# Jittor/JDet

Hardware: AMD Instinct MI355X
Metric: img/s S2ANet-R50-FPN train step, 1024x1024 synthetic tiles (higher is better)
Workload: dtype f32; 1 GPU; s2anet_train; model=S2ANet-R50-FPN (configs/s2anet/s2anet_r50_fpn_1x_dota.py), global_batch=2, tile=1024x1024, gts_per_image=64, optimizer=SGD mom 0.9 wd 1e-4 clip 35 + StepLR warm-up (the config's lr), parallelism=dp1 (DDP, RCCL all-reduce)

## Files before the change

### jdet_amd/_lib.py

```python
import ctypes
import os
import subprocess

import torch

_HERE = os.path.dirname(os.path.abspath(__file__))
CSRC = os.path.join(_HERE, "csrc")
LIB_PATH = os.path.join(CSRC, "libjdet_hip.so")

_i, _f, _p, _sz, _l = ctypes.c_int, ctypes.c_float, ctypes.c_void_p, ctypes.c_size_t, ctypes.c_long



class BnParams(ctypes.Structure):
    _fields_ = [("weight", _p), ("bias", _p), ("mean", _p), ("var", _p), ("eps", _f)]


class ConvEpilogue(ctypes.Structure):
    _fields_ = [("mode", _i), ("affine", _i), ("relu", _i), ("bn", BnParams), ("residual", _p), ("grad_out", _p),
                ("act", _p), ("sums", _p)]


class BnSumsJob(ctypes.Structure):
    _fields_ = [("partial", _p), ("rows", _l), ("C", _i), ("gamma", _p), ("grad_gamma", _p), ("grad_beta", _p)]
# ... 85 lines not shown
                                      _p, _p, _p, _sz, _p]),
    "jdet_level_pack_nhwc": (_i, [_p, _p, _p, _i, _i, _i, _i, _i, _p, _p]),
    "jdet_align_conv_offset": (_i, [_p, _i, _i, _i, _f, _i, _p, _p]),
    "jdet_frozen_bn_act_forward": (_i, [_p, _p, _l, _i, _p, _p, _p, _p, _f, _i, _p, _p]),
    "jdet_frozen_bn_act_backward_workspace": (_sz, [_l, _i]),
    "jdet_frozen_bn_act_backward": (_i, [_p, _p, _p, _l, _i, _p, _p, _p, _p, _f, _i, _p, _p, _p, _p, _p, _sz, _p]),
    "jdet_bias_act_backward": (_i, [_p, _p, _l, _i, _i, _p, _p, _p, _sz, _p]),
    "jdet_channel_sum_workspace": (_sz, [_l, _i]),
    "jdet_channel_sum": (_i, [_p, _l, _i, _p, _p, _sz, _p]),
    "jdet_arf_forward": (_i, [_p, _p] + [_i] * 6 + [_p, _p]),
    "jdet_arf_backward": (_i, [_p, _p] + [_i] * 6 + [_p, _p]),
    "jdet_arf_forward_cl": (_i, [_p, _p] + [_i] * 6 + [_p, _p]),
    "jdet_arf_backward_cl": (_i, [_p, _p] + [_i] * 6 + [_p, _p]),
    "jdet_rip_forward": (_i, [_p, _l, _i, _i, _p, _p]),
    "jdet_rip_backward": (_i, [_p, _p, _p, _l, _i, _i, _p, _p]),
    "jdet_delta2bbox_rotated": (_i, [_p, _p, _i, _i, _p, _p, _f, _p, _p]),
    "jdet_bbox2delta_rotated": (_i, [_p, _p, _i, _p, _p, _p, _p]),
    "jdet_midpoint_offset_decode": (_i, [_p, _p, _l, _p, _p, _f, _p, _p]),
    "jdet_midpoint_offset_encode": (_i, [_p, _p, _l, _p, _p, _p, _p]),
    "jdet_oriented_delta_decode": (_i, [_p, _p, _l, _i, _p, _p, _f, _p, _p]),
    "jdet_oriented_delta_encode": (_i, [_p, _p, _l, _p, _p, _p, _p]),
    "jdet_gliding_targets": (_i, [_p, _p, _l, _p, _p, _p, _p, _p, _p]),
    "jdet_gliding_decode": (_i, [_p, _p, _p, _p, _l, _i, _p, _p, _f, _f, _f, _f, _p, _p, _p]),
    "jdet_gv_delta_encode": (_i, [_p, _p, _l, _p, _p, _p, _p]),
    "jdet_gv_delta_decode": (_i, [_p, _p, _l, _i, _p, _p, _f, _f, _f, _p, _p]),
    "jdet_anchor_targets_rotated": (_i, [_p, _p, _p, _p, _i, _i, _p, _p, _f, _p, _p, _p, _p, _p, _p]),
    "jdet_anchor_targets_rotated_boxes": (_i, [_p, _p, _p, _i, _i, _f, _p, _p, _p, _p, _p, _p]),
    "jdet_obb2hbb2obb": (_i, [_p, _i, _i, _p, _p]),
    "jdet_assign_max_iou_workspace": (_sz, [_i]),
    "jdet_assign_max_iou": (_i, [_p, _i, _i, _f, _f, _f, _f, _i, _i, _p, _i, _p, _p, _p, _p, _sz, _p]),
}

ATSS_SIGNATURES = {
    "jdet_atss_assign_workspace": (_sz, [_i, _i, _i, _i]),
    "jdet_atss_assign": (_i, [_p, _i, _i, _p, _i, _p, _i, _p, _p, _i, _i, _p, _p, _p, _p, _sz, _p]),
}

ROWS_SIGNATURES = {
    "jdet_rows_nonzero_workspace": (_sz, [_i, _i, _i]),
    "jdet_rows_nonzero": (_i, [_p, _i, _i, _i, _i, _p, _p, _p, _p, _p, _sz, _p]),
    "jdet_conv3x3_rows_supported": (_i, [_i, _i]),
    "jdet_conv3x3_wgrad_rows_workers": (_i, [_i, _i]),
    "jdet_conv3x3_wgrad_rows": (_i, [_p, _p, _p, _p, _i, _i, _i, _i, _i, _p, _p]),
    "jdet_conv3x3_dgrad_rows": (_i, [_p, _p, _p, _p, _i, _i, _i, _i, _i, _i, _p, _p]),
}

ROWS_FWD_SIGNATURES = {
    "jdet_rows_from_flags_workspace": (_sz, [_i, _i, _i]),
    "jdet_rows_from_flags": (_i, [_p, _i, _i, _i, _p, _p, _p, _p, _p, _sz, _p]),
    "jdet_conv3x3_rows_forward_supported": (_i, [_i, _i]),
    "jdet_conv3x3_rows_forward": (_i, [_p, _p, _p, _i, _p, _p, _p, _i, _i, _i, _i, _i, _i, _p, _p]),
}

FCOS_SIGNATURES = {
    "jdet_fcos_targets": (_i, [_p, _p, _i, _p, _p, _p, _i, _i, _i, _i, _i, _f, _p, _p, _p, _p, _p]),
    "jdet_poly_iou_loss": (_i, [_p, _p, _p, _l, _i, _f, _p, _p, _p]),
}

REPPOINTS_SIGNATURES = {
    "jdet_convex_point_assign_workspace": (_sz, [_i, _i]),
    "jdet_convex_point_assign": (_i, [_p, _i, _i, _p, _p, _i, _p, _p, _p, _i, _i, _f, _i, _i, _p, _p, _p, _sz, _p]),
    "jdet_convex_giou_loss": (_i, [_p, _p, _p, _p, _l, _p, _p, _p]),
}

H2RBOX_SIGNATURES = {
    "jdet_rotate_crop": (_i, [_p, _i, _i, _i, _i, _i, _i, _f, _f, _i, _p, _p]),
    "jdet_h2rbox_aug_loss_forward": (_i, [_p, _i, _p, _p, _p, _p, _p, _i, _i, _f, _f, _f, _i, _i, _f, _f, _f, _p, _p, _p]),
    "jdet_h2rbox_aug_loss_backward": (_i, [_p, _i, _p, _p, _p, _p, _p, _i, _i, _f, _f, _f, _i, _i, _f, _f, _f, _p, _p, _p,
                                           _p, _p, _p, _p, _p]),
}

_lib = None

REFERENCE_SORT = 0


def build(force=False, verbose=False):
    cmd = ["make", "-C", CSRC, "-j8"] + (["-B"] if force else [])
    r = subprocess.run(cmd, capture_output=True, text=True)
    if r.returncode != 0:
        raise RuntimeError("building libjdet_hip.so failed:\n" + r.stdout[-4000:] + r.stderr[-4000:])
    if verbose:
        print(r.stdout[-2000:])
    return LIB_PATH


def lib():
    global _lib
    if _lib is None:
        if not os.path.exists(LIB_PATH):
            raise RuntimeError(
                "jdet_amd: %s not found.  Build it with `python -c 'import __graft_entry__ as g; g.build()'` "
                "or `make -C jdet_amd/csrc` (needs hipcc).  There is no CPU fallback." % LIB_PATH)
        l = ctypes.CDLL(LIB_PATH)
        for name, (res, args) in list(SIGNATURES.items()) + list(ATSS_SIGNATURES.items()) + list(ROWS_SIGNATURES.items()) + \
                list(ROWS_FWD_SIGNATURES.items()) + list(FCOS_SIGNATURES.items()) + list(REPPOINTS_SIGNATURES.items()) + \
                list(H2RBOX_SIGNATURES.items()):
            fn = getattr(l, name)
            fn.restype = res
            fn.argtypes = args
        _lib = l
    return _lib


class JDetHipError(RuntimeError):
    pass


_ERR = {-1: "bad argument", -2: "unsupported shape", -3: "workspace too small"}


def check(status, what):
    if status != 0:
        msg = _ERR.get(status, "hipError_t %d" % status)
        raise JDetHipError("%s failed: %s" % (what, msg))


def stream_ptr(t=None):
    if t is not None and t.is_cuda and t.device.index != torch.cuda.current_device():
        torch.cuda.set_device(t.device)
    return torch.cuda.current_stream(t.device if t is not None else None).cuda_stream


def need_device(*tensors):
    for t in tensors:
        if t is None:
            continue
        if not t.is_cuda:
            raise JDetHipError(
                "jdet_amd ops run only on a HIP device (got a %s tensor); there is no CPU fallback "
                "in the product path" % t.device)


def f32c(t):
    if t.dtype != torch.float32:
        t = t.float()
    return t.contiguous()


def vec5(v):
    return (ctypes.c_float * 5)(*[float(x) for x in v])


def vecn(v, n):
    v = [float(x) for x in v]
    assert len(v) == n
    return (ctypes.c_float * n)(*v)


def ptr(t):
# ... 33 lines not shown
```

### jdet_amd/csrc/conv_rows.hip

```cpp
#include "conv_mfma.h"
#include "jdet_hip_rows.h"
#include "jdet_hip_rows_fwd.h"

namespace {

constexpr int kBlk = 256;
constexpr int kFlagRows = 64;

typedef unsigned v4u __attribute__((ext_vector_type(4)));

__global__ __launch_bounds__(256) void rows_flag_kernel(const float* __restrict__ g, long P, int C4,
                                                        uint8_t* __restrict__ flags) {
  const int lane = threadIdx.x & 63, wave = threadIdx.x >> 6;
  const long base = (long)blockIdx.x * kFlagRows + wave * (kFlagRows / 4);
  const v4u* g4 = reinterpret_cast<const v4u*>(g);
  for (int r = 0; r < kFlagRows / 4; r += 4) {
    unsigned acc[4] = {0u, 0u, 0u, 0u};
#pragma unroll
    for (int u = 0; u < 4; u++) {
      const long row = base + r + u;
      if (row < P)
        for (int c = lane; c < C4; c += 64) {
          const v4u v = g4[row * C4 + c];
          acc[u] |= (v[0] | v[1] | v[2] | v[3]) & 0x7fffffffu;
        }
    }
#pragma unroll
    for (int u = 0; u < 4; u++) {
      const long row = base + r + u;
      const bool any = __ballot(acc[u] != 0u) != 0ull;
      if (lane == 0 && row < P) flags[row] = any ? 1 : 0;
    }
  }
}

__device__ __forceinline__ int wave_sum(int v) {
#pragma unroll
  for (int o = 32; o > 0; o >>= 1) v += __shfl_xor(v, o, 64);
  return v;
}

__global__ __launch_bounds__(256) void rows_dilate_kernel(const uint8_t* __restrict__ flags, int H, int W, long P,
                                                          uint8_t* __restrict__ dflags, int* __restrict__ cnt,
                                                          int* __restrict__ dcnt) {
  __shared__ int s_sum[2][4];
  const int tid = threadIdx.x, lane = tid & 63, wave = tid >> 6;
  const long p = (long)blockIdx.x * kBlk + tid;
  bool f = false, d = false;
  if (p < P) {
    f = flags[p] != 0;
    const unsigned hw = (unsigned)(H * W), up = (unsigned)p;
    const unsigned rem = up - (up / hw) * hw;
    const int y = (int)(rem / (unsigned)W), x = (int)(rem - (unsigned)y * (unsigned)W);
#pragma unroll
    for (int dy = -1; dy <= 1; dy++)
// ... 189 lines not shown
#pragma unroll
    for (int q = 0; q < BK / 2; q++) {
      if (q + 1 < BK / 2) frags(q + 1);
#pragma unroll
      for (int i = 0; i < TM; i++)
#pragma unroll
        for (int j = 0; j < TN; j++)
          acc[i][j] = __builtin_amdgcn_mfma_f32_32x32x2f32(fa[q & 1][i], fb[q & 1][j], acc[i][j], 0, 0, 0);
    }
    store_step(buf ^ 1);
    __syncthreads();
  }

  const long gw_bytes = (long)a.Cout * 9 * a.Cin * 4;
  if (m0 + BM <= a.Cout && n0 + BN <= a.Cin && gw_bytes < (1L << 32)) {
    const __amdgpu_buffer_rsrc_t rgw = __builtin_amdgcn_make_buffer_rsrc((void*)a.gw, 0, (unsigned)gw_bytes, 0x00020000);
    const unsigned row_bytes = (unsigned)(9 * a.Cin * 4);
#pragma unroll
    for (int i = 0; i < TM; i++)
#pragma unroll
      for (int j = 0; j < TN; j++) {
        const unsigned ci = (unsigned)(n0 + wn * 32 * TN + j * 32 + (lane & 31));
        const unsigned co = (unsigned)(m0 + wm * 32 * TM + i * 32 + 4 * (lane >> 5));
        const unsigned base = ((co * 9u + (unsigned)tap) * (unsigned)a.Cin + ci) * 4u;
#pragma unroll
        for (int e = 0; e < 16; e++)
          __builtin_amdgcn_raw_ptr_buffer_atomic_fadd_f32(acc[i][j][e], rgw, (int)base, (int)(cd_row(e) * row_bytes), 0);
      }
    return;
  }
#pragma unroll
  for (int i = 0; i < TM; i++)
#pragma unroll
    for (int j = 0; j < TN; j++) {
      const int ci = n0 + wn * 32 * TN + j * 32 + (lane & 31);
#pragma unroll
      for (int e = 0; e < 16; e++) {
        const int co = m0 + wm * 32 * TM + i * 32 + cd_row(e) + 4 * (lane >> 5);
        if (co < a.Cout && ci < a.Cin) unsafeAtomicAdd(a.gw + ((size_t)co * 9 + tap) * a.Cin + ci, acc[i][j][e]);
      }
    }
}

struct DgradRowsArgs {
  const float* g;
  const float* wd;
  const int* rows;
  const int* count;
  float* gx;
  int N, H, W, Cin, Cout;
  const float* bias;
  const float* rowmask;
  int relu;
};

template <int BK, int KG, bool FWD>
__global__ __launch_bounds__(256 * KG) __attribute__((amdgpu_waves_per_eu(4)))
void conv3x3_dgrad_rows_kernel(DgradRowsArgs a) {
  constexpr int BT = 64;
  constexpr int DEPTH = KG >= 1 ? 1 : 2;
  using TL = MfmaTile<BT, BK, KG>;
  constexpr int T = TL::T, CH = TL::CH, RPP = TL::RPP, PASSES = TL::PASSES, TILE = TL::TILE, QN = TL::QN;
  static_assert(T == 1, "64 x 64 tile");
  __shared__ __attribute__((aligned(16))) char s_raw[4 * TILE];
  const int tid = threadIdx.x, lane = tid & 63, wave = tid >> 6;
  const int P = a.N * a.H * a.W;
  const int KC = a.Cout, NO = a.Cin;
  int cnt = a.count[0];
  cnt = cnt < 0 ? 0 : (cnt > P ? P : cnt);
  const int NT = (NO + BT - 1) / BT;
  const int mtile = (int)((unsigned)blockIdx.x / (unsigned)NT);
  const int m0 = mtile * BT;
  if (m0 >= cnt) return;
  const int n0 = (blockIdx.x - mtile * NT) * BT;
  const __amdgpu_buffer_rsrc_t rx =
      __builtin_amdgcn_make_buffer_rsrc((void*)a.g, 0, (unsigned)((long)P * KC * 4), 0x00020000);
  const __amdgpu_buffer_rsrc_t rw =
      __builtin_amdgcn_make_buffer_rsrc((void*)a.wd, 0, (unsigned)((long)NO * 9 * KC * 4), 0x00020000);
  const int lchunk = tid % CH, lrow = tid / CH;
  int img[PASSES], py[PASSES], px[PASSES];
  bool m_ok[PASSES];
  unsigned wv[PASSES];
  int st_off[PASSES];
  const unsigned hw = (unsigned)(a.H * a.W);
#pragma unroll
  for (int p = 0; p < PASSES; p++) {
    const int row = p * RPP + lrow;
    const int li = m0 + row;
    const unsigned pos = li < cnt ? (unsigned)a.rows[li] : 0xFFFFFFFFu;
    m_ok[p] = pos < (unsigned)P;
    const unsigned im = m_ok[p] ? pos / hw : 0u, rem = m_ok[p] ? pos - im * hw : 0u, oy = rem / (unsigned)a.W;
    img[p] = (int)im;
    py[p] = (int)oy;
    px[p] = (int)(rem - oy * (unsigned)a.W);
    wv[p] = n0 + row < NO ? ((unsigned)((n0 + row) * 9 * KC + lchunk * 4)) * 4u : kOob;
    st_off[p] = swz_bytes<BK>(row, lchunk);
  }
  const int nsteps = 9 * (KC / BK);

  unsigned av[PASSES];
  auto set_tap = [&](int tap) {
    const int r = (tap * 11) >> 5, s = tap - r * 3;
#pragma unroll
    for (int p = 0; p < PASSES; p++) {
      const int yy = py[p] + r - 1, xx = px[p] + s - 1;
      const bool in = m_ok[p] && (unsigned)yy < (unsigned)a.H && (unsigned)xx < (unsigned)a.W;
      const unsigned off = ((unsigned)(((img[p] * a.H + yy) * a.W + xx) * KC + lchunk * 4)) * 4u;
      av[p] = in ? off : kOob;
    }
  };

  v4f ra[DEPTH][PASSES], rb[DEPTH][PASSES];
  auto load_set = [&](auto setc, int tap, int c) {
    constexpr int S = decltype(setc)::value;
    const unsigned sa = (unsigned)(c * 4), sb = (unsigned)((tap * KC + c) * 4);
#pragma unroll
    for (int p = 0; p < PASSES; p++) {
      ra[S][p] = buf_load(rx, av[p], sa);
      rb[S][p] = buf_load(rw, wv[p], sb);
    }
  };
  auto store_set = [&](auto setc, int buf) {
    constexpr int S = decltype(setc)::value;
#pragma unroll
    for (int p = 0; p < PASSES; p++) {
      *reinterpret_cast<v4f*>(s_raw + buf * 2 * TILE + st_off[p]) = ra[S][p];
      *reinterpret_cast<v4f*>(s_raw + buf * 2 * TILE + TILE + st_off[p]) = rb[S][p];
    }
  };
  auto load_step = [&](int tap, int c) { load_set(Set0{}, tap, c); };
  auto store_step = [&](int buf) { store_set(Set0{}, buf); };

  const int kg = wave >> 2, wm = (wave >> 1) & 1, wn = wave & 1;
  const int frow = lane & 31, fhalf = lane >> 5;
  int fa_off[QN], fb_off[QN];
#pragma unroll
  for (int qq = 0; qq < QN; qq++) {
    const int chunk = (qq * KG + kg) * 2 + fhalf;
    fa_off[qq] = swz_bytes<BK>(wm * (BT / 2) + frow, chunk);
    fb_off[qq] = TILE + swz_bytes<BK>(wn * (BT / 2) + frow, chunk);
  }
  v16f acc[T][T];
#pragma unroll
  for (int e = 0; e < 16; e++) acc[0][0][e] = 0.f;

  int tap = 0, c = 0;
  set_tap(0);
  auto advance = [&]() {
    c += BK;
    if (c == KC) {
      c = 0;
      tap++;
      set_tap(tap);
    }
  };
  auto mfma_step = [&](int buf) { ::mfma_step<BT, BK, KG>(s_raw, buf, fa_off, fb_off, acc); };
#include "conv_mfma_loop.inc"
  if (KG == 2) {
    float* red = reinterpret_cast<float*>(s_raw);
    if (kg == 1) {
#pragma unroll
      for (int e = 0; e < 16; e++) red[red_index<T>(wave, lane, 0, 0, e)] = acc[0][0][e];
    }
    __syncthreads();
    if (kg == 1) return;
  }

  const __amdgpu_buffer_rsrc_t ry =
      __builtin_amdgcn_make_buffer_rsrc((void*)a.gx, 0, (unsigned)((long)P * NO * 4), 0x00020000);
  const int lrow0 = m0 + wm * (BT / 2) + 4 * (lane >> 5);
  const int n = n0 + wn * (BT / 2) + (lane & 31);
  unsigned dst[16];
  float mk[16];
  float b = 0.f;
  if constexpr (FWD) b = (a.bias && n < NO) ? a.bias[n] : 0.f;
#pragma unroll
  for (int e = 0; e < 16; e++) {
    const int li = lrow0 + cd_row(e);
    const unsigned pos = li < cnt ? (unsigned)a.rows[li] : 0xFFFFFFFFu;
    dst[e] = (pos < (unsigned)P && n < NO) ? (pos * (unsigned)NO + (unsigned)n) * 4u : kOob;
    if constexpr (FWD) mk[e] = (a.rowmask && pos < (unsigned)P) ? a.rowmask[pos] : 1.f;
  }
#pragma unroll
  for (int e = 0; e < 16; e++) {
    float v = acc[0][0][e];
    if (KG == 2) v += reinterpret_cast<const float*>(s_raw)[red_index<T>(wave, lane, 0, 0, e)];
    if constexpr (FWD) {
      v += b;
      if (a.relu) v = fmaxf(v, 0.f);
      if (a.rowmask) v *= mk[e];
    }
    __builtin_amdgcn_raw_buffer_store_b32(__builtin_bit_cast(unsigned, v), ry, dst[e], 0u, 0);
  }
}

inline size_t align16(size_t v) { return (v + 15) & ~(size_t)15; }

inline int wgrad_rows_workers(int Cin, int Cout) {
  const int tm = Cout > 64 ? 2 : 1;
  const long tiles = (long)((Cout + 64 * tm - 1) / (64 * tm)) * ((Cin + 63) / 64) * 9;
  long kw = 1152 / tiles;
  return (int)(kw < 8 ? 8 : (kw > 64 ? 64 : kw));
}

}

JDET_API size_t jdet_rows_nonzero_workspace(int N, int H, int W) {
  if (N <= 0 || H <= 0 || W <= 0) return 0;
  const long P = (long)N * H * W;
  const long nb = (P + kBlk - 1) / kBlk;
  return align16((size_t)P) + sizeof(int32_t) * 2 * (size_t)nb;
}

JDET_API int jdet_rows_nonzero(const float* g_nhwc, int N, int H, int W, int C, uint8_t* flags, int32_t* rows,
                               int32_t* rows_dilated, int32_t* counts, void* workspace, size_t workspace_bytes,
                               jdet_stream_t stream) {
  if (N <= 0 || H <= 0 || W <= 0 || C <= 0) return JDET_E_BADARG;
  if (C % 4 != 0) return JDET_E_UNSUPPORTED;
  const long P = (long)N * H * W;
  if (P * C >= (1L << 30)) return JDET_E_UNSUPPORTED;
  if (!g_nhwc || !flags || !rows || !rows_dilated || !counts) return JDET_E_BADARG;
  if (((uintptr_t)g_nhwc & 15) || (((uintptr_t)rows | (uintptr_t)rows_dilated | (uintptr_t)counts) & 3))
    return JDET_E_BADARG;
  if (!workspace || workspace_bytes < jdet_rows_nonzero_workspace(N, H, W)) return JDET_E_WORKSPACE;
  if ((uintptr_t)workspace & 3) return JDET_E_BADARG;
  hipStream_t st = (hipStream_t)stream;
  const unsigned nb = (unsigned)((P + kBlk - 1) / kBlk);
  uint8_t* dflags = (uint8_t*)workspace;
  int* cnt = (int*)((char*)workspace + align16((size_t)P));
  int* dcnt = cnt + nb;
  hipLaunchKernelGGL(rows_flag_kernel, dim3((unsigned)((P + kFlagRows - 1) / kFlagRows)), dim3(256), 0, st, g_nhwc, P,
                     C / 4, flags);
  hipLaunchKernelGGL(rows_dilate_kernel, dim3(nb), dim3(256), 0, st, flags, H, W, P, dflags, cnt, dcnt);
  hipLaunchKernelGGL(rows_list_kernel, dim3(nb), dim3(256), 0, st, flags, dflags, P, cnt, dcnt, rows, rows_dilated,
                     counts);
  return jdet_launch_status();
}

JDET_API int jdet_conv3x3_rows_supported(int Cin, int Cout) {
  return Cin > 0 && Cout > 0 && Cin % 4 == 0 && Cout % 16 == 0;
}

JDET_API int jdet_conv3x3_wgrad_rows_workers(int Cin, int Cout) {
  return jdet_conv3x3_rows_supported(Cin, Cout) ? wgrad_rows_workers(Cin, Cout) : 0;
}

JDET_API int jdet_conv3x3_wgrad_rows(const float* x_nhwc, const float* gy_nhwc, const int32_t* rows,
                                     const int32_t* count, int N, int H, int W, int Cin, int Cout, float* gw_krsc,
                                     jdet_stream_t stream) {
  if (N <= 0 || H <= 0 || W <= 0 || Cin <= 0 || Cout <= 0) return JDET_E_BADARG;
  if (!jdet_conv3x3_rows_supported(Cin, Cout)) return JDET_E_UNSUPPORTED;
  const long P = (long)N * H * W;
  if ((P + BKW) * (Cin > Cout ? Cin : Cout) >= (1L << 30)) return JDET_E_UNSUPPORTED;
  if (!x_nhwc || !gy_nhwc || !rows || !count || !gw_krsc) return JDET_E_BADARG;
  if ((((uintptr_t)x_nhwc) | ((uintptr_t)gy_nhwc)) & 15 || (((uintptr_t)rows | (uintptr_t)count) & 3)) return JDET_E_BADARG;
  const int tm = Cout > 64 ? 2 : 1;
  const int kw = wgrad_rows_workers(Cin, Cout);
  const unsigned grid = (unsigned)(((Cout + 64 * tm - 1) / (64 * tm)) * ((Cin + 63) / 64) * 9 * kw);
  WgradRowsArgs a{x_nhwc, gy_nhwc, rows, count, gw_krsc, N, H, W, Cin, Cout, kw};
  hipStream_t st = (hipStream_t)stream;
  if (tm == 2) hipLaunchKernelGGL((conv3x3_wgrad_rows_kernel<2>), dim3(grid), dim3(256), 0, st, a);
  else hipLaunchKernelGGL((conv3x3_wgrad_rows_kernel<1>), dim3(grid), dim3(256), 0, st, a);
  return jdet_launch_status();
}

JDET_API int jdet_conv3x3_dgrad_rows(const float* gy_nhwc, const float* wd_crsk, const int32_t* rows,
                                     const int32_t* count, int N, int H, int W, int Cin, int Cout, int zero_first,
                                     float* gx_nhwc, jdet_stream_t stream) {
  if (N <= 0 || H <= 0 || W <= 0 || Cin <= 0 || Cout <= 0) return JDET_E_BADARG;
  if (!jdet_conv3x3_rows_supported(Cin, Cout)) return JDET_E_UNSUPPORTED;
  const long P = (long)N * H * W;
  if (P * (Cin > Cout ? Cin : Cout) >= (1L << 30)) return JDET_E_UNSUPPORTED;
  if (!gy_nhwc || !wd_crsk || !rows || !count || !gx_nhwc) return JDET_E_BADARG;
  if ((((uintptr_t)gy_nhwc) | ((uintptr_t)wd_crsk)) & 15 || (((uintptr_t)rows | (uintptr_t)count | (uintptr_t)gx_nhwc) & 3))
    return JDET_E_BADARG;
  hipStream_t st = (hipStream_t)stream;
  if (zero_first) {
    const int e = jdet_zero_async(gx_nhwc, sizeof(float) * (size_t)P * Cin, st);
    if (e) return e;
  }
  DgradRowsArgs a{gy_nhwc, wd_crsk, rows, count, gx_nhwc, N, H, W, Cin, Cout, nullptr, nullptr, 0};
  const unsigned grid = (unsigned)(((P + 63) / 64) * ((Cin + 63) / 64));
  if (Cout % 32 == 0) hipLaunchKernelGGL((conv3x3_dgrad_rows_kernel<32, 2, false>), dim3(grid), dim3(512), 0, st, a);
  else hipLaunchKernelGGL((conv3x3_dgrad_rows_kernel<16, 1, false>), dim3(grid), dim3(256), 0, st, a);
  return jdet_launch_status();
}


JDET_API size_t jdet_rows_from_flags_workspace(int N, int H, int W) {
  if (N <= 0 || H <= 0 || W <= 0) return 0;
  const long P = (long)N * H * W;
  const long nb = (P + kBlk - 1) / kBlk;
  return 2 * align16((size_t)P) + sizeof(int32_t) * 4 * (size_t)nb;
}

JDET_API int jdet_rows_from_flags(const uint8_t* flags, int N, int H, int W, int32_t* rows, int32_t* rows_dilated,
                                  int32_t* rows_dilated2, int32_t* counts, void* workspace, size_t workspace_bytes,
                                  jdet_stream_t stream) {
  if (N <= 0 || H <= 0 || W <= 0) return JDET_E_BADARG;
  const long P = (long)N * H * W;
  if (P >= (1L << 30)) return JDET_E_UNSUPPORTED;
  if (!flags || !rows || !rows_dilated || !rows_dilated2 || !counts) return JDET_E_BADARG;
  if (((uintptr_t)rows | (uintptr_t)rows_dilated | (uintptr_t)rows_dilated2 | (uintptr_t)counts) & 3) return JDET_E_BADARG;
  if (!workspace || workspace_bytes < jdet_rows_from_flags_workspace(N, H, W)) return JDET_E_WORKSPACE;
  if ((uintptr_t)workspace & 3) return JDET_E_BADARG;
  hipStream_t st = (hipStream_t)stream;
  const unsigned nb = (unsigned)((P + kBlk - 1) / kBlk);
  uint8_t* d1 = (uint8_t*)workspace;
  uint8_t* d2 = d1 + align16((size_t)P);
  int* c0 = (int*)(d2 + align16((size_t)P));
  int* c1 = c0 + nb;
  int* c1b = c1 + nb;
  int* c2 = c1b + nb;
  hipLaunchKernelGGL(rows_dilate_kernel, dim3(nb), dim3(256), 0, st, flags, H, W, P, d1, c0, c1);
  hipLaunchKernelGGL(rows_dilate_kernel, dim3(nb), dim3(256), 0, st, (const uint8_t*)d1, H, W, P, d2, c1b, c2);
  hipLaunchKernelGGL(rows_list_kernel, dim3(nb), dim3(256), 0, st, flags, (const uint8_t*)d1, P, (const int*)c0,
                     (const int*)c1, rows, rows_dilated, counts);
  hipLaunchKernelGGL(rows_list_kernel, dim3(nb), dim3(256), 0, st, (const uint8_t*)d1, (const uint8_t*)d2, P,
                     (const int*)c1b, (const int*)c2, rows_dilated, rows_dilated2, counts + 1);
  return jdet_launch_status();
}

JDET_API int jdet_conv3x3_rows_forward_supported(int Cin, int Cout) {
  return Cin > 0 && Cout > 0 && Cin % 16 == 0 && Cout % 16 == 0;
}

JDET_API int jdet_conv3x3_rows_forward(const float* x_nhwc, const float* w_krsc, const float* bias, int relu,
                                       const float* rowmask, const int32_t* rows, const int32_t* count, int N, int H,
                                       int W, int Cin, int Cout, int zero_first, float* y_nhwc, jdet_stream_t stream) {
  if (N <= 0 || H <= 0 || W <= 0 || Cin <= 0 || Cout <= 0) return JDET_E_BADARG;
  if (!jdet_conv3x3_rows_forward_supported(Cin, Cout)) return JDET_E_UNSUPPORTED;
  const long P = (long)N * H * W;
  if (P * (Cin > Cout ? Cin : Cout) >= (1L << 30)) return JDET_E_UNSUPPORTED;
  if (!x_nhwc || !w_krsc || !rows || !count || !y_nhwc) return JDET_E_BADARG;
  if ((((uintptr_t)x_nhwc) | ((uintptr_t)w_krsc)) & 15) return JDET_E_BADARG;
  if (((uintptr_t)rows | (uintptr_t)count | (uintptr_t)y_nhwc | (uintptr_t)bias | (uintptr_t)rowmask) & 3) return JDET_E_BADARG;
  hipStream_t st = (hipStream_t)stream;
  if (zero_first) {
    const int e = jdet_zero_async(y_nhwc, sizeof(float) * (size_t)P * Cout, st);
    if (e) return e;
  }
  DgradRowsArgs a{x_nhwc, w_krsc, rows, count, y_nhwc, N, H, W, Cout, Cin, bias, rowmask, relu ? 1 : 0};
  const unsigned grid = (unsigned)(((P + 63) / 64) * ((Cout + 63) / 64));
  if (Cin % 32 == 0) hipLaunchKernelGGL((conv3x3_dgrad_rows_kernel<32, 2, true>), dim3(grid), dim3(512), 0, st, a);
  else hipLaunchKernelGGL((conv3x3_dgrad_rows_kernel<16, 1, true>), dim3(grid), dim3(256), 0, st, a);
  return jdet_launch_status();
}
```

### jdet_amd/ops/conv_igemm.py

```python
import os
import weakref

import torch

from jdet_amd import _lib as L


def supported(cin, cout):
    return bool(L.lib().jdet_conv3x3_igemm_supported(int(cin), int(cout)))


def weight_krsc(weight):
    return L.f32c(weight.permute(0, 2, 3, 1))


def conv3x3_nhwc(x_nhwc, w_krsc, bias=None, relu=False, rowmask=None, offset=None, tile=0):
    L.need_device(x_nhwc, w_krsc, bias, rowmask, offset)
    N, H, W, Cin = x_nhwc.shape
    Cout = w_krsc.shape[0]
    if w_krsc.shape[1:] != (3, 3, Cin):
        raise ValueError("weight %r does not match input channels %d" % (tuple(w_krsc.shape), Cin))
    if offset is not None and tuple(offset.shape) != (N, 18, H, W):
        raise ValueError("offset must be (N, 18, H, W), got %r" % (tuple(offset.shape),))
    x_nhwc, w_krsc = L.f32c(x_nhwc), L.f32c(w_krsc)
# ... 146 lines not shown
def _bias_bwd_supported(c):
    q = c // 4
    return c % 4 == 0 and ((q <= 256 and 256 % q == 0) or 256 < q <= 1024)


def bias_act_backward(g, y, relu):
    N, C, H, W = g.shape
    if (BIAS_ACT_BWD and not relu and g.is_cuda and g.dtype == torch.float32 and not _bias_bwd_supported(C)
            and C <= 256 and N * H * W > 0):
        gn = L.f32c(g.permute(0, 2, 3, 1))
        P = N * H * W
        nbytes = L.lib().jdet_channel_sum_workspace(P, C)
        ws = torch.empty((nbytes,), dtype=torch.uint8, device=g.device)
        gb = torch.empty((C,), dtype=torch.float32, device=g.device)
        L.check(L.lib().jdet_channel_sum(L.ptr(gn), P, C, L.ptr(gb), L.ptr(ws), nbytes, L.stream_ptr(gn)),
                "jdet_channel_sum")
        return g, gb
    if not (BIAS_ACT_BWD and g.is_cuda and g.dtype == torch.float32 and _bias_bwd_supported(C) and N * H * W > 0):
        gp = torch.ops.aten.threshold_backward(g, y, 0) if relu else g
        return gp, gp.sum((0, 2, 3))
    gn = L.f32c(g.permute(0, 2, 3, 1))
    P = N * H * W
    nbytes = L.lib().jdet_frozen_bn_act_backward_workspace(P, C)
    if torch.cuda.is_current_stream_capturing():
        ws = torch.empty((max(nbytes, 1),), dtype=torch.uint8, device=g.device)
    else:
        key = (g.device.index, torch.cuda.current_stream(g.device).cuda_stream)
        ws = _BWD_WS.get(key)
        if ws is None or ws.numel() < nbytes:
            while len(_BWD_WS) >= 8:
                _BWD_WS.pop(next(iter(_BWD_WS)))
            ws = _BWD_WS[key] = torch.empty((max(nbytes, 1 << 20),), dtype=torch.uint8, device=g.device)
    gb = torch.empty((C,), dtype=torch.float32, device=g.device)
    gp = torch.empty_like(gn) if relu else gn
    yn = L.f32c(y.permute(0, 2, 3, 1)) if relu else None
    L.check(L.lib().jdet_bias_act_backward(L.ptr(gn), L.ptr(yn), P, C, int(bool(relu)), L.ptr(gp) if relu else None,
                                           L.ptr(gb), L.ptr(ws), ws.numel(), L.stream_ptr(gn)),
            "jdet_bias_act_backward")
    return gp.permute(0, 3, 1, 2), gb


ROWS = os.environ.get("JDET_CONV_ROWS", "1") == "1"
_ROWS_WS = {}


def wgrad_rows_workers(cin, cout):
    return int(L.lib().jdet_conv3x3_wgrad_rows_workers(int(cin), int(cout)))


def rows_supported(cin, cout):
    return bool(L.lib().jdet_conv3x3_rows_supported(int(cin), int(cout)))


def _rows_scratch(nbytes, device):
    if torch.cuda.is_current_stream_capturing():
        return torch.empty((nbytes,), dtype=torch.uint8, device=device)
    key = (device.index, torch.cuda.current_stream(device).cuda_stream)
    ws = _ROWS_WS.get(key)
    if ws is None or ws.numel() < nbytes:
        while len(_ROWS_WS) >= 8:
            _ROWS_WS.pop(next(iter(_ROWS_WS)))
        ws = _ROWS_WS[key] = torch.empty((max(nbytes, 1 << 20),), dtype=torch.uint8, device=device)
    return ws


def rows_nonzero(g_nhwc, scratch=None):
    L.need_device(g_nhwc)
    N, H, W, C = g_nhwc.shape
    P = N * H * W
    g_nhwc = L.f32c(g_nhwc)
    wsb = L.lib().jdet_rows_nonzero_workspace(N, H, W)
    total = 8 * P + 16 + wsb + P
    buf = _rows_scratch(total, g_nhwc.device) if scratch is None else scratch
    rows = buf[:4 * P].view(torch.int32)
    drows = buf[4 * P:8 * P].view(torch.int32)
    counts = buf[8 * P:8 * P + 8].view(torch.int32)
    ws = buf[8 * P + 16:8 * P + 16 + wsb]
    flags = buf[8 * P + 16 + wsb:total]
    L.check(L.lib().jdet_rows_nonzero(L.ptr(g_nhwc), N, H, W, C, L.ptr(flags), L.ptr(rows), L.ptr(drows), L.ptr(counts),
                                      L.ptr(ws), wsb, L.stream_ptr(g_nhwc)), "jdet_rows_nonzero")
    return flags, rows, drows, counts


def conv3x3_dgrad_rows_nhwc(gy_nhwc, wd_crsk, rows, count_ptr, out=None):
    L.need_device(gy_nhwc, wd_crsk, rows, out)
    N, H, W, Cout = gy_nhwc.shape
    Cin = wd_crsk.shape[0]
    if tuple(wd_crsk.shape) != (Cin, 3, 3, Cout) or not wd_crsk.is_contiguous():
        raise ValueError("wd must be a contiguous (Cin, 3, 3, Cout) tensor, got %r" % (tuple(wd_crsk.shape),))
    gy_nhwc = L.f32c(gy_nhwc)
    zero = out is None
    if zero:
        out = torch.empty((N, H, W, Cin), dtype=torch.float32, device=gy_nhwc.device)
    L.check(L.lib().jdet_conv3x3_dgrad_rows(L.ptr(gy_nhwc), L.ptr(wd_crsk), L.ptr(rows), count_ptr, N, H, W, Cin, Cout,
                                            int(zero), L.ptr(out), L.stream_ptr(gy_nhwc)), "jdet_conv3x3_dgrad_rows")
    return out


def _rows_dgrad_weight(weight):
    if torch.cuda.is_current_stream_capturing() or not weight.is_cuda:
        return weight.detach().flip(2, 3).permute(1, 2, 3, 0).contiguous()
    wd = dgrad_weight(weight)
    st = _DGRAD_BANKS.get(weight.device)
    if st is None or st["bank"] is None or id(weight) not in st["items"]:
        return dgrad_weight_fresh(weight)
    tid = torch._C._current_graph_task_id()
    if tid < 0 or st.get("pass") != tid:
        st["bank"].refresh()
        st["pass"] = tid
    return wd


def dgrad_weight_fresh(weight):
    return weight.detach().flip(2, 3).permute(1, 2, 3, 0).contiguous()


def _rows_backward(g, x, weight, need_x, need_w):
    gn, xn = L.f32c(g.permute(0, 2, 3, 1)), L.f32c(x.permute(0, 2, 3, 1))
    _, rows, drows, counts = rows_nonzero(gn)
    gx = gw = None
    if need_w:
        gw = shared_wgrad(weight, xn, gn, rows=(rows, counts.data_ptr()))
    if need_x:
        gx = conv3x3_dgrad_rows_nhwc(gn, _rows_dgrad_weight(weight), drows, counts.data_ptr() + 4).permute(0, 3, 1, 2)
    return gx, gw


ROWS_FWD = os.environ.get("JDET_CONV_ROWS_FWD", "1") == "1"


def rows_forward_supported(cin, cout):
    return bool(L.lib().jdet_conv3x3_rows_forward_supported(int(cin), int(cout)))


def rows_from_flags(flags, N, H, W):
    L.need_device(flags)
    P = N * H * W
    if flags.numel() != P or flags.element_size() != 1 or not flags.is_contiguous():
        raise ValueError("flags must be %d contiguous bytes, got %r %s" % (P, tuple(flags.shape), flags.dtype))
    wsb = L.lib().jdet_rows_from_flags_workspace(N, H, W)
    buf = torch.empty((12 * P + 16 + wsb,), dtype=torch.uint8, device=flags.device)
    rows = [buf[4 * i * P:4 * (i + 1) * P].view(torch.int32) for i in range(3)]
    counts = buf[12 * P:12 * P + 12].view(torch.int32)
    ws = buf[12 * P + 16:]
    L.check(L.lib().jdet_rows_from_flags(L.ptr(flags), N, H, W, L.ptr(rows[0]), L.ptr(rows[1]), L.ptr(rows[2]),
                                         L.ptr(counts), L.ptr(ws), wsb, L.stream_ptr(flags)), "jdet_rows_from_flags")
    return rows[0], rows[1], rows[2], counts


def conv3x3_rows_forward_nhwc(x_nhwc, w_krsc, bias, relu, rowmask, rows, count_ptr, out=None):
    L.need_device(x_nhwc, w_krsc, bias, rowmask, rows, out)
    N, H, W, Cin = x_nhwc.shape
    Cout = w_krsc.shape[0]
    if tuple(w_krsc.shape[1:]) != (3, 3, Cin):
        raise ValueError("weight %r does not match input channels %d" % (tuple(w_krsc.shape), Cin))
    x_nhwc, w_krsc = L.f32c(x_nhwc), L.f32c(w_krsc)
    zero = out is None
    if zero:
        out = torch.empty((N, H, W, Cout), dtype=torch.float32, device=x_nhwc.device)
    L.check(L.lib().jdet_conv3x3_rows_forward(
        L.ptr(x_nhwc), L.ptr(w_krsc), L.ptr(L.f32c(bias)) if bias is not None else None, int(bool(relu)),
        L.ptr(L.f32c(rowmask)) if rowmask is not None else None, L.ptr(rows), count_ptr, N, H, W, Cin, Cout, int(zero),
        L.ptr(out), L.stream_ptr(x_nhwc)), "jdet_conv3x3_rows_forward")
    return out


class _ConvBiasActRows(torch.autograd.Function):

    @staticmethod
    def forward(ctx, x, weight, bias, relu, rowmask, rows, count_ptr):
        y = conv3x3_rows_forward_nhwc(L.f32c(x.permute(0, 2, 3, 1)), weight_krsc(weight), bias, relu, rowmask, rows,
                                      count_ptr).permute(0, 3, 1, 2)
        ctx.k1 = False
        ctx.row_sparse = True
        ctx.cfg = (bool(relu), [1, 1], [1, 1], [1, 1], 1, True, bias is not None)
        ctx.save_for_backward(x, weight, y if relu else None)
        return y

    @staticmethod
    def backward(ctx, g):
        return _ConvBiasAct.backward(ctx, g)[:7]


def rows_tower_applicable(convs, x, positions=None):
    if not (ROWS and ROWS_FWD and TRAIN and BIAS_ACT_BWD and 1 <= len(convs) <= 2):
        return False
    if not (x.is_cuda and x.dtype == torch.float32 and x.dim() == 4) or torch.is_autocast_enabled():
        return False
    for conv in convs:
        if not (type(conv).__name__ == "Conv2d" and conv.padding_mode == "zeros" and not isinstance(conv.padding, str)
                and _is_igemm_conv(conv) and conv.weight.dtype == torch.float32 and conv.bias is not None
                and conv.bias.requires_grad and _bias_bwd_supported(conv.out_channels)
                and rows_forward_supported(conv.in_channels, conv.out_channels)
                and rows_supported(conv.in_channels, conv.out_channels)):
            return False
    P = x.shape[0] * x.shape[2] * x.shape[3] if positions is None else positions
    return (P + 16) * max([c.in_channels for c in convs] + [c.out_channels for c in convs]) < 2 ** 30


def rows_tower(convs, x, flags, rowmask=None):
    N, _, H, W = x.shape
    lists = rows_from_flags(flags, N, H, W)
    counts = lists[3]
    n = len(convs)
    for i, conv in enumerate(convs):
        k = n - i
        x = _ConvBiasActRows.apply(x, conv.weight, conv.bias, True, rowmask, lists[k], counts.data_ptr() + 4 * k)
    return x


CONV1X1_GEMM = os.environ.get("JDET_CONV1X1_GEMM", "1") == "1"


def _is_1x1(x, weight, stride, padding, groups):
    return (CONV1X1_GEMM and tuple(weight.shape[2:]) == (1, 1) and tuple(stride) == (1, 1) and tuple(padding) == (0, 0)
            and groups == 1 and x.is_cuda and x.dtype == torch.float32 and weight.shape[0] >= 64
# ... 120 lines not shown
```

Baseline: 86.88 img/s.

## Split row-sparse 3x3 conv reduction over taps when few rows are active

Adds a split-K variant of the row-sparse 3x3 conv forward and dgrad kernels. When the active row count fits under a cap, each workgroup handles a subset of the 9 taps and writes partial sums to a workspace. A finish kernel then adds the parts and applies bias, ReLU and rowmask. The aim is to fill the GPU when few rows are active, at the cost of an extra launch and a round trip of partial sums through workspace memory. It is enabled by default through an environment flag.

```diff
diff --git a/include/jdet_hip_rows_split.h b/include/jdet_hip_rows_split.h
--- /dev/null
+++ b/include/jdet_hip_rows_split.h
@@ -0,0 +1,28 @@
+#ifndef JDET_HIP_ROWS_SPLIT_H_
+#define JDET_HIP_ROWS_SPLIT_H_
+
+#include "jdet_hip.h"
+
+#ifdef __cplusplus
+extern "C" {
+#endif
+
+int jdet_conv3x3_rows_split_max_rows(int Cin, int Cout);
+
+int jdet_conv3x3_rows_split_parts(void);
+
+size_t jdet_conv3x3_rows_split_workspace(int Cin, int Cout, int max_rows, int parts);
+
+int jdet_conv3x3_dgrad_rows_split(const float* gy_nhwc, const float* wd_crsk, const int32_t* rows, const int32_t* count,
+                                  int N, int H, int W, int Cin, int Cout, int zero_first, float* gx_nhwc, int max_rows,
+                                  int parts, void* workspace, size_t workspace_bytes, jdet_stream_t stream);
+
+int jdet_conv3x3_rows_forward_split(const float* x_nhwc, const float* w_krsc, const float* bias, int relu,
+                                    const float* rowmask, const int32_t* rows, const int32_t* count, int N, int H, int W,
+                                    int Cin, int Cout, int zero_first, float* y_nhwc, int max_rows, int parts,
+                                    void* workspace, size_t workspace_bytes, jdet_stream_t stream);
+
+#ifdef __cplusplus
+}
+#endif
+#endif
diff --git a/jdet_amd/_lib.py b/jdet_amd/_lib.py
--- a/jdet_amd/_lib.py
+++ b/jdet_amd/_lib.py
@@ -161,6 +161,15 @@
     "jdet_conv3x3_rows_forward": (_i, [_p, _p, _p, _i, _p, _p, _p, _i, _i, _i, _i, _i, _i, _p, _p]),
 }
 
+ROWS_SPLIT_SIGNATURES = {
+    "jdet_conv3x3_rows_split_max_rows": (_i, [_i, _i]),
+    "jdet_conv3x3_rows_split_parts": (_i, []),
+    "jdet_conv3x3_rows_split_workspace": (_sz, [_i, _i, _i, _i]),
+    "jdet_conv3x3_dgrad_rows_split": (_i, [_p, _p, _p, _p, _i, _i, _i, _i, _i, _i, _p, _i, _i, _p, _sz, _p]),
+    "jdet_conv3x3_rows_forward_split": (_i, [_p, _p, _p, _i, _p, _p, _p, _i, _i, _i, _i, _i, _i, _p, _i, _i, _p, _sz,
+                                             _p]),
+}
+
 FCOS_SIGNATURES = {
     "jdet_fcos_targets": (_i, [_p, _p, _i, _p, _p, _p, _i, _i, _i, _i, _i, _f, _p, _p, _p, _p, _p]),
     "jdet_poly_iou_loss": (_i, [_p, _p, _p, _l, _i, _f, _p, _p, _p]),
@@ -204,7 +213,7 @@
         l = ctypes.CDLL(LIB_PATH)
         for name, (res, args) in list(SIGNATURES.items()) + list(ATSS_SIGNATURES.items()) + list(ROWS_SIGNATURES.items()) + \
                 list(ROWS_FWD_SIGNATURES.items()) + list(FCOS_SIGNATURES.items()) + list(REPPOINTS_SIGNATURES.items()) + \
-                list(H2RBOX_SIGNATURES.items()):
+                list(H2RBOX_SIGNATURES.items()) + list(ROWS_SPLIT_SIGNATURES.items()):
             fn = getattr(l, name)
             fn.restype = res
             fn.argtypes = args
diff --git a/jdet_amd/csrc/conv_rows.hip b/jdet_amd/csrc/conv_rows.hip
--- a/jdet_amd/csrc/conv_rows.hip
+++ b/jdet_amd/csrc/conv_rows.hip
@@ -1,6 +1,7 @@
 #include "conv_mfma.h"
 #include "jdet_hip_rows.h"
 #include "jdet_hip_rows_fwd.h"
+#include "jdet_hip_rows_split.h"
 
 namespace {
 
@@ -296,9 +297,11 @@
   const float* bias;
   const float* rowmask;
   int relu;
+  int parts, max_rows, cap_tiles;
+  float* ws;
 };
 
-template <int BK, int KG, bool FWD>
+template <int BK, int KG, bool FWD, bool SPLIT = false>
 __global__ __launch_bounds__(256 * KG) __attribute__((amdgpu_waves_per_eu(4)))
 void conv3x3_dgrad_rows_kernel(DgradRowsArgs a) {
   constexpr int BT = 64;
@@ -313,10 +316,22 @@
   int cnt = a.count[0];
   cnt = cnt < 0 ? 0 : (cnt > P ? P : cnt);
   const int NT = (NO + BT - 1) / BT;
-  const int mtile = (int)((unsigned)blockIdx.x / (unsigned)NT);
+  int mtile = (int)((unsigned)blockIdx.x / (unsigned)NT);
+  int ntile = blockIdx.x - mtile * NT;
+  int part = 0;
+  bool split = false;
+  if constexpr (SPLIT) {
+    split = cnt <= a.max_rows;
+    if (split) {
+      const unsigned q = (unsigned)blockIdx.x / (unsigned)a.parts;
+      part = (int)(blockIdx.x - q * (unsigned)a.parts);
+      mtile = (int)(q / (unsigned)NT);
+      ntile = (int)q - mtile * NT;
+    }
+  }
   const int m0 = mtile * BT;
   if (m0 >= cnt) return;
-  const int n0 = (blockIdx.x - mtile * NT) * BT;
+  const int n0 = ntile * BT;
   const __amdgpu_buffer_rsrc_t rx =
       __builtin_amdgcn_make_buffer_rsrc((void*)a.g, 0, (unsigned)((long)P * KC * 4), 0x00020000);
   const __amdgpu_buffer_rsrc_t rw =
@@ -340,7 +355,8 @@
     wv[p] = n0 + row < NO ? ((unsigned)((n0 + row) * 9 * KC + lchunk * 4)) * 4u : kOob;
     st_off[p] = swz_bytes<BK>(row, lchunk);
   }
-  const int nsteps = 9 * (KC / BK);
+  const int taps = (SPLIT && split) ? 9 / a.parts : 9;
+  const int nsteps = taps * (KC / BK);
 
   unsigned av[PASSES];
   auto set_tap = [&](int tap) {
@@ -388,8 +404,8 @@
 #pragma unroll
   for (int e = 0; e < 16; e++) acc[0][0][e] = 0.f;
 
-  int tap = 0, c = 0;
-  set_tap(0);
+  int tap = (SPLIT && split) ? part * taps : 0, c = 0;
+  set_tap(tap);
   auto advance = [&]() {
     c += BK;
     if (c == KC) {
@@ -410,10 +426,27 @@
     if (kg == 1) return;
   }
 
+  const int lrow0 = m0 + wm * (BT / 2) + 4 * (lane >> 5);
+  const int n = n0 + wn * (BT / 2) + (lane & 31);
+  if constexpr (SPLIT) {
+    if (split) {
+      const unsigned cap_pad = (unsigned)(a.cap_tiles * BT);
+      const __amdgpu_buffer_rsrc_t rws = __builtin_amdgcn_make_buffer_rsrc(
+          (void*)a.ws, 0, (unsigned)((long)a.parts * cap_pad * NO * 4), 0x00020000);
+#pragma unroll
+      for (int e = 0; e < 16; e++) {
+        const int li = lrow0 + cd_row(e);
+        float v = acc[0][0][e];
+        if (KG == 2) v += reinterpret_cast<const float*>(s_raw)[red_index<T>(wave, lane, 0, 0, e)];
+        const unsigned off = (li < cnt && n < NO) ? (((unsigned)part * cap_pad + (unsigned)li) * (unsigned)NO + (unsigned)n) * 4u : kOob;
+        __builtin_amdgcn_raw_buffer_store_b32(__builtin_bit_cast(unsigned, v), rws, off, 0u, 0);
+      }
+      return;
+    }
+  }
+
   const __amdgpu_buffer_rsrc_t ry =
       __builtin_amdgcn_make_buffer_rsrc((void*)a.gx, 0, (unsigned)((long)P * NO * 4), 0x00020000);
-  const int lrow0 = m0 + wm * (BT / 2) + 4 * (lane >> 5);
-  const int n = n0 + wn * (BT / 2) + (lane & 31);
   unsigned dst[16];
   float mk[16];
   float b = 0.f;
@@ -438,7 +471,67 @@
   }
 }
 
+template <bool FWD>
+__global__ __launch_bounds__(256) void conv3x3_rows_split_finish_kernel(DgradRowsArgs a) {
+  const int P = a.N * a.H * a.W, NO = a.Cin, C4 = NO >> 2;
+  int cnt = a.count[0];
+  cnt = cnt < 0 ? 0 : (cnt > P ? P : cnt);
+  if (cnt > a.max_rows) return;
+  const unsigned idx = blockIdx.x * 256u + threadIdx.x;
+  const unsigned li = idx / (unsigned)C4, c4 = idx - li * (unsigned)C4;
+  if (li >= (unsigned)cnt) return;
+  const unsigned pos = (unsigned)a.rows[li];
+  if (pos >= (unsigned)P) return;
+  const v4f* w = reinterpret_cast<const v4f*>(a.ws) + (size_t)li * C4 + c4;
+  const size_t stride = (size_t)a.cap_tiles * 64 * C4;
+  v4f t[9];
+#pragma unroll
+  for (int s = 0; s < 9; s++)
+    if (s < a.parts) t[s] = w[s * stride];
+  v4f v = t[0];
+#pragma unroll
+  for (int s = 1; s < 9; s++)
+    if (s < a.parts) v += t[s];
+  if constexpr (FWD) {
+    const float mk = a.rowmask ? a.rowmask[pos] : 1.f;
+#pragma unroll
+    for (int k = 0; k < 4; k++) {
+      float x = v[k] + (a.bias ? a.bias[c4 * 4 + k] : 0.f);
+      if (a.relu) x = fmaxf(x, 0.f);
+      if (a.rowmask) x *= mk;
+      v[k] = x;
+    }
+  }
+  *reinterpret_cast<v4f*>(a.gx + (size_t)pos * NO + c4 * 4) = v;
+}
+
 inline size_t align16(size_t v) { return (v + 15) & ~(size_t)15; }
+
+constexpr int kSplitWorkgroups = 256;
+constexpr int kSplitParts = 9;
+inline int split_max_rows(int NO) { return 64 * ((kSplitWorkgroups + (NO + 63) / 64 - 1) / ((NO + 63) / 64)); }
+inline bool split_parts_ok(int parts) { return parts == 3 || parts == 9; }
+
+struct SplitPlan {
+  int parts, max_rows, cap_tiles;
+  size_t bytes;
+  unsigned grid, finish_grid;
+};
+
+inline bool split_plan(long P, int NO, int parts, int max_rows, SplitPlan* sp) {
+  sp->parts = parts > 0 ? parts : kSplitParts;
+  if (!split_parts_ok(sp->parts)) return false;
+  long mr = max_rows > 0 ? max_rows : split_max_rows(NO);
+  if (mr > P) mr = P;
+  sp->max_rows = (int)mr;
+  sp->cap_tiles = (int)((mr + 63) / 64);
+  const long NT = (NO + 63) / 64, mtiles = (P + 63) / 64;
+  sp->bytes = sizeof(float) * (size_t)sp->parts * sp->cap_tiles * 64 * NO;
+  const long split_ids = sp->cap_tiles * NT * sp->parts, plain_ids = mtiles * NT;
+  sp->grid = (unsigned)(split_ids > plain_ids ? split_ids : plain_ids);
+  sp->finish_grid = (unsigned)(((long)sp->cap_tiles * 64 * (NO / 4) + 255) / 256);
+  return true;
+}
 
 inline int wgrad_rows_workers(int Cin, int Cout) {
   const int tm = Cout > 64 ? 2 : 1;
@@ -523,7 +616,7 @@
     const int e = jdet_zero_async(gx_nhwc, sizeof(float) * (size_t)P * Cin, st);
     if (e) return e;
   }
-  DgradRowsArgs a{gy_nhwc, wd_crsk, rows, count, gx_nhwc, N, H, W, Cin, Cout, nullptr, nullptr, 0};
+  DgradRowsArgs a{gy_nhwc, wd_crsk, rows, count, gx_nhwc, N, H, W, Cin, Cout, nullptr, nullptr, 0, 0, 0, 0, nullptr};
   const unsigned grid = (unsigned)(((P + 63) / 64) * ((Cin + 63) / 64));
   if (Cout % 32 == 0) hipLaunchKernelGGL((conv3x3_dgrad_rows_kernel<32, 2, false>), dim3(grid), dim3(512), 0, st, a);
   else hipLaunchKernelGGL((conv3x3_dgrad_rows_kernel<16, 1, false>), dim3(grid), dim3(256), 0, st, a);
@@ -584,9 +677,83 @@
     const int e = jdet_zero_async(y_nhwc, sizeof(float) * (size_t)P * Cout, st);
     if (e) return e;
   }
-  DgradRowsArgs a{x_nhwc, w_krsc, rows, count, y_nhwc, N, H, W, Cout, Cin, bias, rowmask, relu ? 1 : 0};
+  DgradRowsArgs a{x_nhwc, w_krsc, rows, count, y_nhwc, N, H, W, Cout, Cin, bias, rowmask, relu ? 1 : 0, 0, 0, 0, nullptr};
   const unsigned grid = (unsigned)(((P + 63) / 64) * ((Cout + 63) / 64));
   if (Cin % 32 == 0) hipLaunchKernelGGL((conv3x3_dgrad_rows_kernel<32, 2, true>), dim3(grid), dim3(512), 0, st, a);
   else hipLaunchKernelGGL((conv3x3_dgrad_rows_kernel<16, 1, true>), dim3(grid), dim3(256), 0, st, a);
   return jdet_launch_status();
 }
+
+
+JDET_API int jdet_conv3x3_rows_split_max_rows(int Cin, int Cout) {
+  if (!jdet_conv3x3_rows_supported(Cin, Cout)) return 0;
+  return split_max_rows(Cin > Cout ? Cin : Cout);
+}
+
+JDET_API int jdet_conv3x3_rows_split_parts(void) { return kSplitParts; }
+
+JDET_API size_t jdet_conv3x3_rows_split_workspace(int Cin, int Cout, int max_rows, int parts) {
+  if (!jdet_conv3x3_rows_supported(Cin, Cout)) return 0;
+  if (parts <= 0) parts = kSplitParts;
+  if (!split_parts_ok(parts)) return 0;
+  if (max_rows <= 0) max_rows = jdet_conv3x3_rows_split_max_rows(Cin, Cout);
+  const size_t NO = (size_t)(Cin > Cout ? Cin : Cout);
+  return sizeof(float) * (size_t)parts * (((size_t)max_rows + 63) / 64 * 64) * NO;
+}
+
+namespace {
+
+template <bool FWD>
+int rows_split_launch(DgradRowsArgs a, long P, int parts, int max_rows, void* workspace, size_t workspace_bytes,
+                      int zero_first, hipStream_t st) {
+  const int NO = a.Cin, KC = a.Cout;
+  SplitPlan sp;
+  if (!split_plan(P, NO, parts, max_rows > 0 ? max_rows : split_max_rows(NO > KC ? NO : KC), &sp)) return JDET_E_BADARG;
+  if (sp.bytes >= ((size_t)1 << 32)) return JDET_E_UNSUPPORTED;
+  if (!workspace || workspace_bytes < sp.bytes / NO * (NO > KC ? NO : KC)) return JDET_E_WORKSPACE;
+  if (((uintptr_t)workspace | (uintptr_t)a.gx) & 15) return JDET_E_BADARG;
+  if (zero_first) {
+    const int e = jdet_zero_async(a.gx, sizeof(float) * (size_t)P * NO, st);
+    if (e) return e;
+  }
+  a.parts = sp.parts;
+  a.max_rows = sp.max_rows;
+  a.cap_tiles = sp.cap_tiles;
+  a.ws = (float*)workspace;
+  if (KC % 32 == 0) hipLaunchKernelGGL((conv3x3_dgrad_rows_kernel<32, 2, FWD, true>), dim3(sp.grid), dim3(512), 0, st, a);
+  else hipLaunchKernelGGL((conv3x3_dgrad_rows_kernel<16, 1, FWD, true>), dim3(sp.grid), dim3(256), 0, st, a);
+  hipLaunchKernelGGL((conv3x3_rows_split_finish_kernel<FWD>), dim3(sp.finish_grid), dim3(256), 0, st, a);
+  return jdet_launch_status();
+}
+
+}
+
+JDET_API int jdet_conv3x3_dgrad_rows_split(const float* gy_nhwc, const float* wd_crsk, const int32_t* rows,
+                                           const int32_t* count, int N, int H, int W, int Cin, int Cout, int zero_first,
+                                           float* gx_nhwc, int max_rows, int parts, void* workspace,
+                                           size_t workspace_bytes, jdet_stream_t stream) {
+  if (N <= 0 || H <= 0 || W <= 0 || Cin <= 0 || Cout <= 0 || max_rows < 0 || parts < 0) return JDET_E_BADARG;
+  if (!jdet_conv3x3_rows_supported(Cin, Cout)) return JDET_E_UNSUPPORTED;
+  const long P = (long)N * H * W;
+  if (P * (Cin > Cout ? Cin : Cout) >= (1L << 30)) return JDET_E_UNSUPPORTED;
+  if (!gy_nhwc || !wd_crsk || !rows || !count || !gx_nhwc) return JDET_E_BADARG;
+  if ((((uintptr_t)gy_nhwc) | ((uintptr_t)wd_crsk)) & 15 || (((uintptr_t)rows | (uintptr_t)count) & 3)) return JDET_E_BADARG;
+  DgradRowsArgs a{gy_nhwc, wd_crsk, rows, count, gx_nhwc, N, H, W, Cin, Cout, nullptr, nullptr, 0, 0, 0, 0, nullptr};
+  return rows_split_launch<false>(a, P, parts, max_rows, workspace, workspace_bytes, zero_first, (hipStream_t)stream);
+}
+
+JDET_API int jdet_conv3x3_rows_forward_split(const float* x_nhwc, const float* w_krsc, const float* bias, int relu,
+                                             const float* rowmask, const int32_t* rows, const int32_t* count, int N,
+                                             int H, int W, int Cin, int Cout, int zero_first, float* y_nhwc,
+                                             int max_rows, int parts, void* workspace, size_t workspace_bytes,
+                                             jdet_stream_t stream) {
+  if (N <= 0 || H <= 0 || W <= 0 || Cin <= 0 || Cout <= 0 || max_rows < 0 || parts < 0) return JDET_E_BADARG;
+  if (!jdet_conv3x3_rows_forward_supported(Cin, Cout)) return JDET_E_UNSUPPORTED;
+  const long P = (long)N * H * W;
+  if (P * (Cin > Cout ? Cin : Cout) >= (1L << 30)) return JDET_E_UNSUPPORTED;
+  if (!x_nhwc || !w_krsc || !rows || !count || !y_nhwc) return JDET_E_BADARG;
+  if ((((uintptr_t)x_nhwc) | ((uintptr_t)w_krsc)) & 15) return JDET_E_BADARG;
+  if (((uintptr_t)rows | (uintptr_t)count | (uintptr_t)bias | (uintptr_t)rowmask) & 3) return JDET_E_BADARG;
+  DgradRowsArgs a{x_nhwc, w_krsc, rows, count, y_nhwc, N, H, W, Cout, Cin, bias, rowmask, relu ? 1 : 0, 0, 0, 0, nullptr};
+  return rows_split_launch<true>(a, P, parts, max_rows, workspace, workspace_bytes, zero_first, (hipStream_t)stream);
+}
diff --git a/jdet_amd/ops/conv_igemm.py b/jdet_amd/ops/conv_igemm.py
--- a/jdet_amd/ops/conv_igemm.py
+++ b/jdet_amd/ops/conv_igemm.py
@@ -222,13 +222,13 @@
     return bool(L.lib().jdet_conv3x3_rows_supported(int(cin), int(cout)))
 
 
-def _rows_scratch(nbytes, device):
+def _rows_scratch(nbytes, device, use="lists"):
     if torch.cuda.is_current_stream_capturing():
         return torch.empty((nbytes,), dtype=torch.uint8, device=device)
-    key = (device.index, torch.cuda.current_stream(device).cuda_stream)
+    key = (use, device.index, torch.cuda.current_stream(device).cuda_stream)
     ws = _ROWS_WS.get(key)
     if ws is None or ws.numel() < nbytes:
-        while len(_ROWS_WS) >= 8:
+        while len(_ROWS_WS) >= 16:
             _ROWS_WS.pop(next(iter(_ROWS_WS)))
         ws = _ROWS_WS[key] = torch.empty((max(nbytes, 1 << 20),), dtype=torch.uint8, device=device)
     return ws
@@ -252,7 +252,23 @@
     return flags, rows, drows, counts
 
 
-def conv3x3_dgrad_rows_nhwc(gy_nhwc, wd_crsk, rows, count_ptr, out=None):
+ROWS_KSPLIT = os.environ.get("JDET_CONV_ROWS_KSPLIT", "1") == "1"
+
+
+def rows_split_max_rows(cin, cout):
+    return int(L.lib().jdet_conv3x3_rows_split_max_rows(int(cin), int(cout)))
+
+
+def _rows_split_ws(cin, cout, positions, device, max_rows=0, parts=0):
+    cap = max_rows if max_rows > 0 else rows_split_max_rows(cin, cout)
+    nbytes = int(L.lib().jdet_conv3x3_rows_split_workspace(int(cin), int(cout), min(cap, positions), int(parts)))
+    if nbytes == 0:
+        raise L.JDetHipError("jdet_conv3x3_rows_split_workspace: unsupported channels %d -> %d or parts %d"
+                             % (cin, cout, parts))
+    return _rows_scratch(nbytes, device, "split"), nbytes
+
+
+def conv3x3_dgrad_rows_nhwc(gy_nhwc, wd_crsk, rows, count_ptr, out=None, split=None, max_rows=0, parts=0):
     L.need_device(gy_nhwc, wd_crsk, rows, out)
     N, H, W, Cout = gy_nhwc.shape
     Cin = wd_crsk.shape[0]
@@ -262,6 +278,12 @@
     zero = out is None
     if zero:
         out = torch.empty((N, H, W, Cin), dtype=torch.float32, device=gy_nhwc.device)
+    if ROWS_KSPLIT if split is None else split:
+        ws, nbytes = _rows_split_ws(Cin, Cout, N * H * W, gy_nhwc.device, max_rows, parts)
+        L.check(L.lib().jdet_conv3x3_dgrad_rows_split(
+            L.ptr(gy_nhwc), L.ptr(wd_crsk), L.ptr(rows), count_ptr, N, H, W, Cin, Cout, int(zero), L.ptr(out),
+            int(max_rows), int(parts), L.ptr(ws), nbytes, L.stream_ptr(gy_nhwc)), "jdet_conv3x3_dgrad_rows_split")
+        return out
     L.check(L.lib().jdet_conv3x3_dgrad_rows(L.ptr(gy_nhwc), L.ptr(wd_crsk), L.ptr(rows), count_ptr, N, H, W, Cin, Cout,
                                             int(zero), L.ptr(out), L.stream_ptr(gy_nhwc)), "jdet_conv3x3_dgrad_rows")
     return out
@@ -318,7 +340,8 @@
     return rows[0], rows[1], rows[2], counts
 
 
-def conv3x3_rows_forward_nhwc(x_nhwc, w_krsc, bias, relu, rowmask, rows, count_ptr, out=None):
+def conv3x3_rows_forward_nhwc(x_nhwc, w_krsc, bias, relu, rowmask, rows, count_ptr, out=None, split=None, max_rows=0,
+                              parts=0):
     L.need_device(x_nhwc, w_krsc, bias, rowmask, rows, out)
     N, H, W, Cin = x_nhwc.shape
     Cout = w_krsc.shape[0]
@@ -328,10 +351,18 @@
     zero = out is None
     if zero:
         out = torch.empty((N, H, W, Cout), dtype=torch.float32, device=x_nhwc.device)
+    bias = L.f32c(bias) if bias is not None else None
+    rowmask = L.f32c(rowmask) if rowmask is not None else None
+    if ROWS_KSPLIT if split is None else split:
+        ws, nbytes = _rows_split_ws(Cin, Cout, N * H * W, x_nhwc.device, max_rows, parts)
+        L.check(L.lib().jdet_conv3x3_rows_forward_split(
+            L.ptr(x_nhwc), L.ptr(w_krsc), L.ptr(bias), int(bool(relu)), L.ptr(rowmask), L.ptr(rows), count_ptr, N, H, W,
+            Cin, Cout, int(zero), L.ptr(out), int(max_rows), int(parts), L.ptr(ws), nbytes, L.stream_ptr(x_nhwc)),
+            "jdet_conv3x3_rows_forward_split")
+        return out
     L.check(L.lib().jdet_conv3x3_rows_forward(
-        L.ptr(x_nhwc), L.ptr(w_krsc), L.ptr(L.f32c(bias)) if bias is not None else None, int(bool(relu)),
-        L.ptr(L.f32c(rowmask)) if rowmask is not None else None, L.ptr(rows), count_ptr, N, H, W, Cin, Cout, int(zero),
-        L.ptr(out), L.stream_ptr(x_nhwc)), "jdet_conv3x3_rows_forward")
+        L.ptr(x_nhwc), L.ptr(w_krsc), L.ptr(bias), int(bool(relu)), L.ptr(rowmask), L.ptr(rows), count_ptr, N, H, W, Cin,
+        Cout, int(zero), L.ptr(out), L.stream_ptr(x_nhwc)), "jdet_conv3x3_rows_forward")
     return out
 
 
```

New measurement: 88.05 img/s, median of 6. 1.01x the previous value.
